# lppllppl920/EndoscopyDepthEstimation-Pytorch

Measured on AMD Instinct MI355X. Metric: train frame-pairs/sec at 256x320 bs=8, higher is better.
Workload: dtype f32

## Files before the change

### endoscopydepthestimation-pytorch_amd/csrc/conv_dma_kernels.h

```cpp
#pragma once

#include "conv_kernels.h"

namespace endo {

static __device__ __attribute__((aligned(16))) float g_pad_consts[8] = {__builtin_nanf(""), __builtin_nanf(""), __builtin_nanf(""), __builtin_nanf(""),
                                                                  0.0f, 0.0f, 0.0f, 0.0f};

typedef const __attribute__((address_space(1))) void* gptr_t;
typedef __attribute__((address_space(3))) void* lptr_t;

template <int KS, int KC, int Q, int WX, int R, int NBUF, int VEC, int IN = IN_PLAIN>
struct ConvDmaSmem {
    using G = ConvGeom<KS, KC, WX, R, VEC>;
    static constexpr int kW = KS * KS * KC * 16 * Q;
    static constexpr int kUG = (G::kTileX / 2) * (G::kTileY / 2);
    static constexpr int kUI = kUG / 4;
    static constexpr int kUStride = ((kUG + kUI - 8 + 31) / 32) * 32 + 8;
    static constexpr int kChan = (IN == IN_UNPOOL) ? kUStride : G::kCS;
    static constexpr int kBuf = KC * kChan + kW;
    static constexpr int kTail = 4 * 16 * Q + 8 * 16 * Q;
    static size_t bytes(int bn_cap) { return sizeof(float) * (NBUF * kBuf + 3 * bn_cap + kTail); }
};

template <int KS, int KC, int Q, int IN, int EPI, int WX, int R, int NBUF, int MINW, int VEC, int XF, int EXP = 0, int PH = -1, int BF = 0>
__global__ void __launch_bounds__(kConvThreads, MINW) conv_dma_kernel(const ConvParams p0) {
    static_assert(BF == 0 || (PH < 0 && (KS == 3 || KS == 1) && (IN == IN_BNRELU || IN == IN_PLAIN || (IN == IN_UNPOOL && KS == 1))),
                  "bf16 operands: the ordinary 3x3 convolution and the 1x1 convolutions of the transition-down layers");
    static_assert(PH < 0 || (KS == 3 && (Q % 2) == 0 && IN == IN_PLAIN && EPI == EPI_FWD), "phase mode is the transition-up forward");
    static_assert(IN != IN_UNPOOL || (KS == 1 && R % 2 == 0), "UNPOOL is the transition-down data gradient (1x1)");
    static_assert(NBUF == 1 || NBUF == 2, "one or two LDS buffers");
    static_assert(VEC == 1 || (VEC == 4 && IN != IN_UPSAMPLE && IN != IN_UNPOOL && IN != IN_SUBPIX), "16-byte DMA needs contiguous sources");
    static_assert(IN != IN_SUBPIX || (KS == 3 && EPI == EPI_FWD && PH < 0), "sub-pixel input mode is the transition-up data gradient");
    using G = ConvGeom<KS, KC, WX, R, VEC>;
    using S = ConvDmaSmem<KS, KC, Q, WX, R, NBUF, VEC, IN>;
    constexpr int KK = KS * KS;
    constexpr int NB = 16 * Q;
    constexpr int kWElems = S::kW;
    constexpr int kWPre = (kWElems + kConvThreads - 1) / kConvThreads;
    constexpr bool kDgrad = (EPI == EPI_DGRAD_BN || EPI == EPI_DGRAD_SUMPOOL);
    constexpr int kPhW = 2 * 12 * 16 + 16;
    static_assert(PH < 0 || KC * kPhW <= kWElems, "the phase weights fit the ordinary weight buffer");
    constexpr int kSubW = 4 * 16 * Q + 16;

    extern __shared__ __attribute__((aligned(16))) float smem[];
    float* s_aux = smem + NBUF * S::kBuf;
    int grp, n;
    group_of(p0, blockIdx.z, grp, n);
    const ConvParams p = group_view(p0, grp);
    const int groups = p0.group_n > 0 ? gridDim.z / p0.group_n : 1;
    const bool first_of_group = blockIdx.x == 0 && blockIdx.y == 0 && n == 0;
    (void)groups; (void)first_of_group;
    const int cap = p.bn_cap;

    const int tid = threadIdx.x;
    const int lane = tid & 63;
    const int wave = __builtin_amdgcn_readfirstlane(tid >> 6);
    const int tile = (gridDim.x & 7) == 0 ? xcd_remap(blockIdx.x, gridDim.x) : blockIdx.x;
    const int x0 = (tile % p.tiles_x) * G::kTileX;
    const int y0 = (tile / p.tiles_x) * G::kTileY;
    const int ph = PH == 2 ? static_cast<int>(blockIdx.y) : PH;
    const int co_base = (p.ksplit > 0 || PH == 2) ? 0 : blockIdx.y * NB;

    if constexpr (IN == IN_BNRELU) {
        for (int c = tid; c < p.cin; c += kConvThreads) {
            float scale, mean, beta;
            bn_input_constants(p, p0, grp, groups, first_of_group, c, scale, mean, beta);
            s_aux[c] = scale;
            s_aux[cap + c] = mean;
            s_aux[2 * cap + c] = beta;
        }
        for (int c = p.cin + tid; c < ((p.cin + KC - 1) / KC) * KC; c += kConvThreads) {
            s_aux[c] = 0.f; s_aux[cap + c] = 0.f; s_aux[2 * cap + c] = 0.f;
        }
    }
    if constexpr (EPI == EPI_DGRAD_BN) {
        float* cst = s_aux + 3 * cap;
        if (tid < NB) {
            const int c = co_base + tid;
            float mean = 0.f, rstd = 0.f, scale = 0.f, beta = 0.f;
            if (c < p.cout) {
                mean = p.bn_saved[2 * c];
                rstd = p.bn_saved[2 * c + 1];
                scale = p.bn_gamma[c] * rstd;
                beta = p.bn_beta[c];
            }
            cst[4 * tid] = scale; cst[4 * tid + 1] = beta; cst[4 * tid + 2] = mean; cst[4 * tid + 3] = rstd;
        }
    }

    f32x4 acc[R][Q];
#pragma unroll
    for (int r = 0; r < R; ++r)
#pragma unroll
        for (int q = 0; q < Q; ++q) acc[r][q] = f32x4{0.f, 0.f, 0.f, 0.f};

    const int wx = (wave % WX) * 16;
    const int wy = (wave / WX) * R;
    const int li = lane & 15;
    const int lk = lane >> 4;

    int goff[G::kPos];
    unsigned pos_ok = 0;
#pragma unroll
    for (int k = 0; k < G::kPos; ++k) {
        const int e = tid + k * kConvThreads;
        goff[k] = 0;
        if (e < G::kUnits) {
            const int ry = e / (G::kCols / VEC);
            const int rx = (e - ry * (G::kCols / VEC)) * VEC;
            const int gy = y0 - G::kHalo + ry;
            const int gx = x0 - G::kLeft + rx;
            if (gy >= 0 && gy < p.h && gx >= 0 && gx < p.w) {
                pos_ok |= (1u << k);
                if constexpr (IN == IN_UPSAMPLE) goff[k] = (gy >> 1) * p.in_w + (gx >> 1);
                else if constexpr (IN == IN_SUBPIX) goff[k] = 2 * gy * p.in_w + 2 * gx;
                else goff[k] = gy * p.in_w + gx;
            }
        }
    }
    constexpr int kUSlots = (IN == IN_UNPOOL) ? (KC * S::kUStride + kConvThreads - 1) / kConvThreads : 1;
    int uoff[kUSlots];
    if constexpr (IN == IN_UNPOOL) {
        constexpr int PC = G::kTileX / 2;
        const int ph = p.h >> 1, pw = p.w >> 1;
#pragma unroll
        for (int k = 0; k < kUSlots; ++k) {
            const int e = tid + k * kConvThreads;
            const int u = e % S::kUStride;
            int off = -1;
            if (e < KC * S::kUStride) {
                if (u < S::kUG) {
                    const int gy = (y0 >> 1) + u / PC, gx = (x0 >> 1) + u % PC;
                    if (gy < ph && gx < pw) off = gy * p.in_w + gx;
                } else if (u < S::kUG + S::kUI) {
                    const int q = u - S::kUG;
                    const int gy = (y0 >> 1) + q / (PC / 4), gx = (x0 >> 1) + 4 * (q % (PC / 4));
                    if (gy < ph && gx < pw) off = gy * p.in_w + gx;
                }
            }
            uoff[k] = off;
        }
    }
    const float* in_n = p.in + n * p.in_ns;
    const float* pad_in = g_pad_consts + (IN == IN_BNRELU ? 0 : 4);
    const float* pad_zero = g_pad_consts + 4;
    const int nchunks_all = (p.cin + KC - 1) / KC;
    int chunk_begin = 0, nchunks = nchunks_all;
    ConvParams po = p;
    if (p.ksplit > 0) {
        const int per = (nchunks_all + p.ksplit - 1) / p.ksplit;
        chunk_begin = blockIdx.y * per;
        nchunks = min(nchunks_all, chunk_begin + per);
        po.out = p.out + blockIdx.y * p.split_stride;
    }

    auto issue_dma = [&](int chunk, int buf) {
        const int c_base = chunk * KC;
        float* s_in = smem + buf * S::kBuf;
        float* s_w = s_in + KC * S::kChan;
        if constexpr (IN == IN_UNPOOL) {
            const uint8_t* idx_n = p.in_idx + n * p.idx_ns;
#pragma unroll
            for (int k = 0; k < kUSlots; ++k) {
                const int e0 = k * kConvThreads + wave * 64;
                if (e0 < KC * S::kUStride) {
                    const int e = e0 + lane;
                    const int ch = c_base + e / S::kUStride;
                    const bool is_code = (e % S::kUStride) >= S::kUG;
                    const void* src = pad_zero;
                    if (uoff[k] >= 0 && ch < p.cin) {
                        const int64_t o = static_cast<int64_t>(ch) * p.in_cs + uoff[k];
                        src = is_code ? static_cast<const void*>(idx_n + o) : static_cast<const void*>(in_n + o);
                    }
                    if (e < KC * S::kUStride) __builtin_amdgcn_global_load_lds((gptr_t)src, (lptr_t)(s_in + e0), 4, 0, 0);
                }
            }
        }
        int sub_ph = 0;
        if constexpr (IN == IN_SUBPIX) sub_ph = c_base / p.sub_c;
#pragma unroll
        for (int c = 0; c < (IN == IN_UNPOOL ? 0 : KC); ++c) {
            const int ch = c_base + c;
            const float* plane = in_n + static_cast<int64_t>(ch) * p.in_cs;
            if constexpr (IN == IN_SUBPIX)
                plane = in_n + static_cast<int64_t>(ch - sub_ph * p.sub_c) * p.in_cs + (sub_ph >> 1) * p.in_w + (sub_ph & 1);
#pragma unroll
            for (int k = 0; k < G::kPos; ++k) {
                const int e0 = k * kConvThreads + wave * 64;
                if (e0 < G::kUnits) {
                    const bool ok = (ch < p.cin) && (pos_ok & (1u << k));
                    const float* src = ok ? plane + goff[k] : pad_in;
                    if (e0 + lane < G::kUnits) {
                        if constexpr (VEC == 4)
                            __builtin_amdgcn_global_load_lds((gptr_t)src, (lptr_t)(s_in + c * G::kCS + 4 * e0), 16, 0, 0);
                        else
                            __builtin_amdgcn_global_load_lds((gptr_t)src, (lptr_t)(s_in + c * G::kCS + e0), 4, 0, 0);
                    }
                }
            }
        }
        if constexpr (IN == IN_SUBPIX) {
            constexpr int kUnitsW = KC * kSubW / 4;
            const float* wsrc = p.wgt + static_cast<int64_t>(c_base) * kSubW;
#pragma unroll
            for (int k = 0; k < (kUnitsW + kConvThreads - 1) / kConvThreads; ++k) {
                const int u0 = k * kConvThreads + wave * 64;
                if (u0 < kUnitsW && u0 + lane < kUnitsW)
                    __builtin_amdgcn_global_load_lds((gptr_t)(wsrc + 4 * (u0 + lane)), (lptr_t)(s_w + 4 * u0), 16, 0, 0);
            }
        }
        if constexpr (PH >= 0) {
            constexpr int kUnitsW = KC * kPhW / 4;
            const float* wsrc = p.wgt + static_cast<int64_t>(c_base) * kPhW + (PH == 2 ? static_cast<int64_t>(ph) * p.cin * 400 : 0);
#pragma unroll
            for (int k = 0; k < (kUnitsW + kConvThreads - 1) / kConvThreads; ++k) {
                const int u0 = k * kConvThreads + wave * 64;
                if (u0 < kUnitsW && u0 + lane < kUnitsW)
                    __builtin_amdgcn_global_load_lds((gptr_t)(wsrc + 4 * (u0 + lane)), (lptr_t)(s_w + 4 * u0), 16, 0, 0);
            }
        }
        constexpr bool kChunked = KS == 3 && KC == 16 && Q == 1 && EPI == EPI_FWD && PH < 0 && IN != IN_SUBPIX && BF == 0;
        bool gather = !(PH >= 0 || IN == IN_SUBPIX);
        if constexpr (kChunked) {
            if (p.wgt_chunks) {
                gather = false;
                constexpr int kUnitsW = kWElems / 4;
                const float* wsrc = p.wgt_chunks + static_cast<int64_t>(chunk) * kWElems;
#pragma unroll
                for (int k = 0; k < (kUnitsW + kConvThreads - 1) / kConvThreads; ++k) {
                    const int u0 = k * kConvThreads + wave * 64;
                    if (u0 < kUnitsW && u0 + lane < kUnitsW)
                        __builtin_amdgcn_global_load_lds((gptr_t)(wsrc + 4 * (u0 + lane)), (lptr_t)(s_w + 4 * u0), 16, 0, 0);
                }
            }
        }
        if (gather)
#pragma unroll
        for (int k = 0; k < ((PH >= 0 || IN == IN_SUBPIX) ? 0 : kWPre); ++k) {
            const int e0 = k * kConvThreads + wave * 64;
            if (e0 < kWElems) {
                const int e = e0 + lane;
                const int j = e % NB;
                const int rest = e / NB;
                const int c = rest % KC;
                const int tap = rest / KC;
                const int ci = c_base + c;
                const int co = co_base + j;
                const float* src = pad_zero;
                if (e < kWElems && ci < p.cin && co < (PH >= 0 ? p.w_cout : p.cout)) {
                    if constexpr (kDgrad) src = p.wgt + (static_cast<int64_t>(ci) * p.w_cin + co) * KK + (KK - 1 - tap);
                    else src = p.wgt + (static_cast<int64_t>(co) * p.w_cin + ci) * KK + tap;
                }
                if (e < kWElems) __builtin_amdgcn_global_load_lds((gptr_t)src, (lptr_t)(s_w + e0), 4, 0, 0);
            }
        }
    };

    constexpr int PR = (EPI == EPI_DGRAD_BN) ? R : 1, PQ = (EPI == EPI_DGRAD_BN) ? Q : 1;
    f32x4 xpre[PR][PQ], dpre[PR][PQ];
    bool use_pre = false;
    if constexpr (EPI == EPI_DGRAD_BN) {
        use_pre = ((p.out_w & 3) == 0) && ((p.w & 3) == 0);
        if (use_pre) {
            const int px = x0 + wx + 4 * lk;
#pragma unroll
            for (int q = 0; q < Q; ++q) {
                const int co = co_base + q * 16 + li;
#pragma unroll
                for (int r = 0; r < R; ++r) {
                    const int y = y0 + wy + r;
                    xpre[r][q] = f32x4{0.f, 0.f, 0.f, 0.f};
                    dpre[r][q] = f32x4{0.f, 0.f, 0.f, 0.f};
                    if (co < p.cout && y < p.h && px + 3 < p.w) {
                        xpre[r][q] = *reinterpret_cast<const f32x4*>(p.x + n * p.x_ns + static_cast<int64_t>(co) * p.x_cs + y * p.out_w + px);
                        if (co >= p.acc_from)
                            dpre[r][q] = *reinterpret_cast<const f32x4*>(p.out + n * p.out_ns + static_cast<int64_t>(co) * p.out_cs + y * p.out_w + px);
                    }
                }
            }
        }
    }

    constexpr bool kInPlace = (IN == IN_BNRELU) && (XF == 1);
    auto transform_own = [&](int chunk, int buf) {
        if constexpr (kInPlace) {
            float* s_in = smem + buf * S::kBuf;
#pragma unroll
            for (int c = 0; c < KC; ++c) {
                const int ch = chunk * KC + c;
                const float sc = s_aux[ch], mn = s_aux[cap + ch], bt = s_aux[2 * cap + ch];
#pragma unroll
                for (int k = 0; k < G::kPos; ++k) {
                    const int e = tid + k * kConvThreads;
                    if (e < G::kUnits) {
                        if constexpr (VEC == 4) {
                            f32x4* q = reinterpret_cast<f32x4*>(s_in + c * G::kCS + 4 * e);
                            f32x4 v = *q;
#pragma unroll
                            for (int i = 0; i < 4; ++i) v[i] = __builtin_fmaxf(fmaf(v[i] - mn, sc, bt), 0.f);
                            *q = v;
                        } else {
                            float* q = s_in + c * G::kCS + e;
                            *q = __builtin_fmaxf(fmaf(*q - mn, sc, bt), 0.f);
                        }
                    }
                }
            }
        }
    };

    auto compute = [&](int chunk, int buf) {
        const float* s_in = smem + buf * S::kBuf;
        const float* s_w = s_in + KC * S::kChan;
        int sub_alpha = 0, sub_beta = 0;
        if constexpr (IN == IN_SUBPIX) {
            const int sub_ph = (chunk * KC) / p.sub_c;
            sub_alpha = sub_ph >> 1; sub_beta = sub_ph & 1;
        }
        (void)sub_alpha; (void)sub_beta;
        if constexpr (IN == IN_UNPOOL) {
            constexpr int PC = G::kTileX / 2;
            const int pcol = (wx + li) >> 1;
            const unsigned sh = 8u * (pcol & 3);
            const unsigned want = li & 1;
            if constexpr (BF != 0) {
                constexpr int NQ = KC / 4;
#pragma unroll
                for (int qg = 0; qg < (NQ + 3) / 4; ++qg) {
                    float a[4][R], b[4][Q];
#pragma unroll
                    for (int i = 0; i < 4; ++i) {
                        const int quad = qg * 4 + i;
                        if (quad < NQ) {
                            const float* g_base = s_in + (quad * 4 + lk) * S::kUStride + (wy >> 1) * PC + pcol;
                            const unsigned* i_base = reinterpret_cast<const unsigned*>(s_in + (quad * 4 + lk) * S::kUStride + S::kUG);
                            const float* b_base = s_w + (quad * 4 + lk) * NB + li;
#pragma unroll
                            for (int rr = 0; rr < R / 2; ++rr) {
                                const float g = g_base[rr * PC];
                                const unsigned code = (i_base[(((wy >> 1) + rr) * PC + pcol) >> 2] >> sh) & 0xffu;
                                a[i][2 * rr] = code == want ? g : 0.f;
                                a[i][2 * rr + 1] = code == want + 2u ? g : 0.f;
                            }
#pragma unroll
                            for (int q = 0; q < Q; ++q) b[i][q] = b_base[q * 16];
                        } else {
#pragma unroll
                            for (int r = 0; r < R; ++r) a[i][r] = 0.f;
#pragma unroll
                            for (int q = 0; q < Q; ++q) b[i][q] = 0.f;
                        }
                    }
                    bf16x4_bits ap[R];
#pragma unroll
                    for (int r = 0; r < R; ++r) ap[r] = pack_bf16x4(a[0][r], a[1][r], a[2][r], a[3][r]);
#pragma unroll
                    for (int q = 0; q < Q; ++q) {
                        const bf16x4_bits bp = pack_bf16x4(b[0][q], b[1][q], b[2][q], b[3][q]);
#pragma unroll
                        for (int r = 0; r < R; ++r) acc[r][q] = __builtin_amdgcn_mfma_f32_16x16x16bf16_1k(ap[r], bp, acc[r][q], 0, 0, 0);
                    }
                }
                return;
            }
#pragma unroll
            for (int quad = 0; quad < KC / 4; ++quad) {
                const float* g_base = s_in + (quad * 4 + lk) * S::kUStride + (wy >> 1) * PC + pcol;
                const unsigned* i_base = reinterpret_cast<const unsigned*>(s_in + (quad * 4 + lk) * S::kUStride + S::kUG);
                const float* b_base = s_w + (quad * 4 + lk) * NB + li;
                float a[R];
#pragma unroll
                for (int rr = 0; rr < R / 2; ++rr) {
                    const float g = g_base[rr * PC];
                    const unsigned code = (i_base[(((wy >> 1) + rr) * PC + pcol) >> 2] >> sh) & 0xffu;
                    a[2 * rr] = code == want ? g : 0.f;
                    a[2 * rr + 1] = code == want + 2u ? g : 0.f;
                }
#pragma unroll
                for (int q = 0; q < Q; ++q) {
                    const float b = b_base[q * 16];
#pragma unroll
                    for (int r = 0; r < R; ++r) acc[r][q] = __builtin_amdgcn_mfma_f32_16x16x4f32(a[r], b, acc[r][q], 0, 0, 0);
                }
            }
            return;
        }
        if constexpr (BF != 0 && KS == 1) {
            constexpr int NQ = KC / 4;
#pragma unroll
            for (int qg = 0; qg < (NQ + 3) / 4; ++qg) {
                float a[4][R], b[4][Q];
#pragma unroll
                for (int i = 0; i < 4; ++i) {
                    const int quad = qg * 4 + i;
                    if (quad < NQ) {
                        const float* a_base = s_in + (quad * 4 + lk) * G::kCS + wy * G::kCols + wx + li + G::kColOff;
                        const float* b_base = s_w + (quad * 4 + lk) * NB + li;
                        float sc = 1.f, mn = 0.f, bt = 0.f;
                        if constexpr (IN == IN_BNRELU && !kInPlace) {
                            const int ch = chunk * KC + quad * 4 + lk;
                            sc = s_aux[ch]; mn = s_aux[cap + ch]; bt = s_aux[2 * cap + ch];
                        }
#pragma unroll
                        for (int r = 0; r < R; ++r) {
                            const float v = a_base[r * G::kCols];
                            a[i][r] = (IN == IN_BNRELU && !kInPlace) ? __builtin_fmaxf(fmaf(v - mn, sc, bt), 0.f) : v;
                        }
#pragma unroll
                        for (int q = 0; q < Q; ++q) b[i][q] = b_base[q * 16];
                    } else {
#pragma unroll
                        for (int r = 0; r < R; ++r) a[i][r] = 0.f;
#pragma unroll
                        for (int q = 0; q < Q; ++q) b[i][q] = 0.f;
                    }
                }
                bf16x4_bits ap[R];
#pragma unroll
                for (int r = 0; r < R; ++r) ap[r] = pack_bf16x4(a[0][r], a[1][r], a[2][r], a[3][r]);
#pragma unroll
                for (int q = 0; q < Q; ++q) {
                    const bf16x4_bits bp = pack_bf16x4(b[0][q], b[1][q], b[2][q], b[3][q]);
#pragma unroll
                    for (int r = 0; r < R; ++r) acc[r][q] = __builtin_amdgcn_mfma_f32_16x16x16bf16_1k(ap[r], bp, acc[r][q], 0, 0, 0);
                }
            }
            return;
        }
#pragma unroll
        for (int quad = 0; quad < KC / 4; ++quad) {
            const float* a_base = s_in + (quad * 4 + lk) * G::kCS + wy * G::kCols + wx + li + G::kColOff;
            const float* b_base = s_w + (quad * 4 + lk) * NB + li;
            float sc = 1.f, mn = 0.f, bt = 0.f;
            if constexpr (IN == IN_BNRELU && !kInPlace) {
                const int ch = chunk * KC + quad * 4 + lk;
                sc = s_aux[ch]; mn = s_aux[cap + ch]; bt = s_aux[2 * cap + ch];
            }
#pragma unroll
            for (int dx = 0; dx < KS; ++dx) {
                float a[R + KS - 1];
                if constexpr (BF != 0) {
#pragma unroll
                    for (int r = 0; r < R + 2; ++r) {
                        const float v = a_base[r * G::kCols + dx];
                        a[r] = (IN == IN_BNRELU && !kInPlace) ? __builtin_fmaxf(fmaf(v - mn, sc, bt), 0.f) : v;
                    }
                    bf16x4_bits ap[R];
#pragma unroll
                    for (int r = 0; r < R; ++r) ap[r] = pack_bf16x4(a[r], a[r + 1], a[r + 2], 0.f);
#pragma unroll
                    for (int q = 0; q < Q; ++q) {
                        const bf16x4_bits bp = pack_bf16x4(b_base[(0 * KS + dx) * KC * NB + q * 16], b_base[(1 * KS + dx) * KC * NB + q * 16],
                                                           b_base[(2 * KS + dx) * KC * NB + q * 16], 0.f);
#pragma unroll
                        for (int r = 0; r < R; ++r) acc[r][q] = __builtin_amdgcn_mfma_f32_16x16x16bf16_1k(ap[r], bp, acc[r][q], 0, 0, 0);
                    }
                    continue;
                }
                if constexpr (IN == IN_BNRELU && !kInPlace && !(EXP & 2)) {
                    typedef float f32x2 __attribute__((ext_vector_type(2)));
                    constexpr int NR = R + KS - 1;
                    const f32x2 mn2 = {mn, mn}, sc2 = {sc, sc}, bt2 = {bt, bt};
#pragma unroll
                    for (int r = 0; r + 1 < NR; r += 2) {
                        f32x2 v = {a_base[r * G::kCols + dx], a_base[(r + 1) * G::kCols + dx]};
                        v = __builtin_elementwise_fma(v - mn2, sc2, bt2);
                        a[r] = __builtin_fmaxf(v[0], 0.f);
                        a[r + 1] = __builtin_fmaxf(v[1], 0.f);
                    }
                    if constexpr (NR & 1) a[NR - 1] = __builtin_fmaxf(fmaf(a_base[(NR - 1) * G::kCols + dx] - mn, sc, bt), 0.f);
                } else {
#pragma unroll
                    for (int r = 0; r < R + KS - 1; ++r) a[r] = a_base[r * G::kCols + dx];
                }
                if constexpr (IN == IN_SUBPIX) {
                    if (dx == (sub_beta == 0 ? 0 : 2)) continue;
                }
#pragma unroll
                for (int dy = 0; dy < KS; ++dy) {
                    if (PH >= 0 && dy == (ph == 0 ? 2 : 0)) continue;
                    if constexpr (IN == IN_SUBPIX) {
                        if (dy == (sub_alpha == 0 ? 0 : 2)) continue;
                    }
#pragma unroll
                    for (int q = 0; q < Q; ++q) {
                        if (PH >= 0 && ((q < Q / 2 && dx == 2) || (q >= Q / 2 && dx == 0))) continue;
                        float b;
                        if constexpr (IN == IN_SUBPIX) {
                            const int tyi = dy - (sub_alpha == 0 ? 1 : 0), txi = dx - (sub_beta == 0 ? 1 : 0);
                            b = s_w[(quad * 4 + lk) * kSubW + (tyi * 2 + txi) * NB + q * 16 + li];
                        } else if constexpr (PH >= 0) {
                            const int slot = dx == 0 ? q : (dx == 1 ? Q / 2 + q : Q / 2 + Q + (q - Q / 2));
                            b = s_w[(quad * 4 + lk) * kPhW + ((dy - ph) * 2 * Q + slot) * 16 + li];
                        } else {
                            b = b_base[(dy * KS + dx) * KC * NB + q * 16];
                        }
#pragma unroll
                        for (int r = 0; r < R; ++r)
                            acc[r][q] = __builtin_amdgcn_mfma_f32_16x16x4f32(a[r + dy], b, acc[r][q], 0, 0, 0);
                    }
                }
            }
        }
    };

    issue_dma(chunk_begin, 0);
    if constexpr (kInPlace) {
        __syncthreads();
        asm volatile("s_waitcnt vmcnt(0)" ::: "memory");
        transform_own(chunk_begin, 0);
        __syncthreads();
        for (int chunk = chunk_begin; chunk < nchunks; ++chunk) {
            const int b = (chunk - chunk_begin) & 1;
            if (chunk + 1 < nchunks) issue_dma(chunk + 1, b ^ 1);
            compute(chunk, b);
            if (chunk + 1 < nchunks) {
                asm volatile("s_waitcnt vmcnt(0)" ::: "memory");
                transform_own(chunk + 1, b ^ 1);
            }
            __syncthreads();
        }
    } else {
        for (int chunk = chunk_begin; chunk < nchunks; ++chunk) {
            const int b = (chunk - chunk_begin) % NBUF;
            if (!(EXP & 4) || chunk == chunk_begin) asm volatile("s_waitcnt vmcnt(0)" ::: "memory");
            __syncthreads();
            if (NBUF == 2 && chunk + 1 < nchunks && !(EXP & 1)) issue_dma(chunk + 1, b ^ 1);
            compute(chunk, b);
            if (NBUF == 1 && chunk + 1 < nchunks) {
                __syncthreads();
                issue_dma(chunk + 1, 0);
            }
        }
    }

    if constexpr (EPI == EPI_DGRAD_BN) {
        if (use_pre) {
            const float* cst = s_aux + 3 * cap;
            float* s_red = s_aux + 3 * cap + 4 * NB;
            const int px = x0 + wx + 4 * lk;
#pragma unroll
            for (int q = 0; q < Q; ++q) {
                const int jloc = q * 16 + li;
                const int co = co_base + jloc;
                const float scale = cst[4 * jloc], beta = cst[4 * jloc + 1], mean = cst[4 * jloc + 2], rstd = cst[4 * jloc + 3];
                float s1 = 0.f, s2 = 0.f;
#pragma unroll
                for (int r = 0; r < R; ++r) {
                    const int y = y0 + wy + r;
                    if (co < p.cout && y < p.h && px + 3 < p.w) {
                        f32x4 o = dpre[r][q];
#pragma unroll
                        for (int e = 0; e < 4; ++e) {
                            const float xc = xpre[r][q][e] - mean;
                            const float z = fmaf(xc, scale, beta);
                            const float dz = z > 0.f ? acc[r][q][e] : 0.f;
                            s1 += dz;
                            s2 += dz * (xc * rstd);
                            o[e] += scale * dz;
                        }
                        *reinterpret_cast<f32x4*>(p.out + n * p.out_ns + static_cast<int64_t>(co) * p.out_cs + y * p.out_w + px) = o;
                    }
                }
                s1 += __shfl_xor(s1, 16, 64); s1 += __shfl_xor(s1, 32, 64);
                s2 += __shfl_xor(s2, 16, 64); s2 += __shfl_xor(s2, 32, 64);
                if (lk == 0) {
                    s_red[((tid >> 6) * NB + jloc) * 2] = s1;
                    s_red[((tid >> 6) * NB + jloc) * 2 + 1] = s2;
                }
            }
            __syncthreads();
            if (tid < 2 * NB) {
                const int j = tid >> 1, which = tid & 1;
                if (co_base + j < p.cout) {
                    double t = 0.0;
                    for (int wv = 0; wv < 4; ++wv) t += static_cast<double>(s_red[(wv * NB + j) * 2 + which]);
                    atomicAdd(p.bn_scratch + bn_slot_offset(p.bn_slot_stride) + 2 * (co_base + j) + which, t);
                }
            }
            return;
        }
    }
    if constexpr (PH >= 0) {
        constexpr int QH = Q / 2;
        float* s_red = s_aux + 3 * cap + 4 * NB;
        const int px = x0 + wx + 4 * lk;
#pragma unroll
        for (int q = 0; q < QH; ++q) {
            const int co = q * 16 + li;
            const bool co_ok = co < p.cout;
            const float bias = (co_ok && p.bias) ? p.bias[co] : 0.f;
            float s1 = 0.f, s2 = 0.f;
#pragma unroll
            for (int r = 0; r < R; ++r) {
                const int y = y0 + wy + r;
                if (co_ok && y < p.h && px + 3 < p.w) {
                    f32x4 lo, hi;
                    lo[0] = acc[r][q][0] + bias; lo[1] = acc[r][q + QH][0] + bias; lo[2] = acc[r][q][1] + bias; lo[3] = acc[r][q + QH][1] + bias;
                    hi[0] = acc[r][q][2] + bias; hi[1] = acc[r][q + QH][2] + bias; hi[2] = acc[r][q][3] + bias; hi[3] = acc[r][q + QH][3] + bias;
                    float* dst = p.out + n * p.out_ns + static_cast<int64_t>(co) * p.out_cs + static_cast<int64_t>(2 * y + ph) * p.out_w + 2 * px;
                    *reinterpret_cast<f32x4*>(dst) = lo;
                    *reinterpret_cast<f32x4*>(dst + 4) = hi;
#pragma unroll
                    for (int e = 0; e < 4; ++e) { s1 += lo[e] + hi[e]; s2 += lo[e] * lo[e] + hi[e] * hi[e]; }
                }
            }
            s1 += __shfl_xor(s1, 16, 64); s1 += __shfl_xor(s1, 32, 64);
            s2 += __shfl_xor(s2, 16, 64); s2 += __shfl_xor(s2, 32, 64);
            if (lk == 0) {
                s_red[((tid >> 6) * NB + q * 16 + li) * 2] = s1;
                s_red[((tid >> 6) * NB + q * 16 + li) * 2 + 1] = s2;
            }
        }
        __syncthreads();
        if (p.out_sums && tid < 2 * 16 * QH) {
            const int j = tid >> 1, which = tid & 1;
            if (j < p.cout) {
                double t = 0.0;
                for (int wv = 0; wv < 4; ++wv) t += static_cast<double>(s_red[(wv * NB + j) * 2 + which]);
                atomicAdd(p.out_sums + 2 * j + which, t);
            }
        }
        return;
    }
    conv_epilogue<Q, EPI, R>(po, acc, s_aux + 3 * cap, s_aux + 3 * cap + 4 * NB, x0, y0, wx, wy, co_base, n);
}

template <int KS, int KC, int Q, int IN, int EPI, int WX, int R, int NBUF, int MINW, int VEC, int XF = 0, int EXP = 0, int PH = -1, int BF = 0>
inline int launch_conv_dma_vec(ConvParams p, hipStream_t stream) {
    static_assert(XF == 0 || NBUF == 2 || IN != IN_BNRELU, "the in-place transform pipeline is written for two buffers");
    using G = ConvGeom<KS, KC, WX, R, VEC>;
    using S = ConvDmaSmem<KS, KC, Q, WX, R, NBUF, VEC, IN>;
    p.tiles_x = (p.w + G::kTileX - 1) / G::kTileX;
    p.bn_cap = (IN == IN_BNRELU) ? ((p.cin + KC - 1) / KC * KC + 15) / 16 * 16 : 0;
    const int tiles_y = (p.h + G::kTileY - 1) / G::kTileY;
    dim3 grid(p.tiles_x * tiles_y, p.ksplit > 0 ? p.ksplit : (PH >= 0 ? (PH == 2 ? 2 : 1) : (p.cout + 16 * Q - 1) / (16 * Q)), p.n);
    return launch_dyn(conv_dma_kernel<KS, KC, Q, IN, EPI, WX, R, NBUF, MINW, VEC, XF, EXP, PH, BF>, grid, kConvThreads, S::bytes(p.bn_cap), stream, p);
}

template <int KS, int KC, int Q, int IN, int EPI, int WX, int R, int NBUF, int MINW = 1, int BF = 0>
inline int launch_conv_dma(const ConvParams& p, hipStream_t stream) {
    if constexpr (IN != IN_UPSAMPLE && IN != IN_UNPOOL) {
        const bool aligned = (p.w % 4 == 0) && (p.in_w % 4 == 0) && (p.in_cs % 4 == 0) && (p.in_ns % 4 == 0) &&
                             (reinterpret_cast<uintptr_t>(p.in) % 16 == 0);
        if (aligned) return launch_conv_dma_vec<KS, KC, Q, IN, EPI, WX, R, NBUF, MINW, 4, 0, 0, -1, BF>(p, stream);
    }
    return launch_conv_dma_vec<KS, KC, Q, IN, EPI, WX, R, NBUF, MINW, 1, 0, 0, -1, BF>(p, stream);
}

template <int KS, int KC, int Q, int IN, int EPI, int BIG_R = 8, int NBUF = 2, int BIG_MINW = 1, int BF = 0>
inline int launch_conv_dma_auto(const ConvParams& p, hipStream_t stream) {
    const long tiles_big = static_cast<long>((p.w + 31) / 32) * ((p.h + 15) / 16) * p.n;
    if (tiles_big >= 512) return launch_conv_dma<KS, KC, Q, IN, EPI, 2, BIG_R, NBUF, BIG_MINW, BF>(p, stream);
    const long tiles_mid = static_cast<long>((p.w + 15) / 16) * ((p.h + 15) / 16) * p.n;
    if (tiles_mid >= 384) return launch_conv_dma<KS, KC, Q, IN, EPI, 1, 4, NBUF, 1, BF>(p, stream);
    constexpr int KCS = (NBUF == 2 && KS == 3 && KC <= 8) ? 16 : KC;
    return launch_conv_dma<KS, KCS, Q, IN, EPI, 1, 2, NBUF, 1, BF>(p, stream);
}

}
```

Baseline: 513.8.

## Pack multi-channel DMA loads for small split-K conv tiles; limit BN constant setup

For ksplit convolutions whose tile has at most 64 vector units per channel, input loads are packed across channels, so each wave issues full 64-lane global_load_lds transfers instead of partially filled per-channel ones. BN-ReLU input constants are now computed only for the channel slice a split block actually uses, not all input channels. Both changes aim to cut wasted DMA issue slots and redundant prologue work in small deep-layer convolutions. The packed path depends on the LDS channel stride equalling the plane size, and adds register pressure from the per-position offset arrays.

Result: no change. 514.5 (median of 6 runs) (+0.1%).

```diff
diff --git a/endoscopydepthestimation-pytorch_amd/csrc/conv_dma_kernels.h b/endoscopydepthestimation-pytorch_amd/csrc/conv_dma_kernels.h
--- a/endoscopydepthestimation-pytorch_amd/csrc/conv_dma_kernels.h
+++ b/endoscopydepthestimation-pytorch_amd/csrc/conv_dma_kernels.h
@@ -63,7 +63,13 @@
     const int co_base = (p.ksplit > 0 || PH == 2) ? 0 : blockIdx.y * NB;
 
     if constexpr (IN == IN_BNRELU) {
-        for (int c = tid; c < p.cin; c += kConvThreads) {
+        int c_lo = 0, c_hi = p.cin;
+        if (p.ksplit > 0 && !first_of_group) {
+            const int per = ((p.cin + KC - 1) / KC + p.ksplit - 1) / p.ksplit * KC;
+            c_lo = min(p.cin, static_cast<int>(blockIdx.y) * per);
+            c_hi = min(p.cin, c_lo + per);
+        }
+        for (int c = c_lo + tid; c < c_hi; c += kConvThreads) {
             float scale, mean, beta;
             bn_input_constants(p, p0, grp, groups, first_of_group, c, scale, mean, beta);
             s_aux[c] = scale;
@@ -119,6 +125,23 @@
             }
         }
     }
+    constexpr bool kPacked = VEC == 4 && KS == 3 && PH < 0 && XF == 0 && (IN == IN_PLAIN || IN == IN_BNRELU) && G::kUnits <= 64 && G::kCS == G::kPlane;
+    constexpr int kPackUnits = KC * G::kUnits;
+    constexpr int kPackPos = kPacked ? (kPackUnits + kConvThreads - 1) / kConvThreads : 1;
+    int pk_off[kPackPos], pk_ch[kPackPos];
+    if constexpr (kPacked) {
+#pragma unroll
+        for (int k = 0; k < kPackPos; ++k) {
+            const int e = tid + k * kConvThreads;
+            const int c = e / G::kUnits, u = e - c * G::kUnits;
+            const int ry = u / (G::kCols / VEC);
+            const int rx = (u - ry * (G::kCols / VEC)) * VEC;
+            const int gy = y0 - G::kHalo + ry;
+            const int gx = x0 - G::kLeft + rx;
+            pk_ch[k] = c;
+            pk_off[k] = (e < kPackUnits && gy >= 0 && gy < p.h && gx >= 0 && gx < p.w) ? c * p.in_cs + gy * p.in_w + gx : -1;
+        }
+    }
     constexpr int kUSlots = (IN == IN_UNPOOL) ? (KC * S::kUStride + kConvThreads - 1) / kConvThreads : 1;
     int uoff[kUSlots];
     if constexpr (IN == IN_UNPOOL) {
@@ -179,6 +202,20 @@
         }
         int sub_ph = 0;
         if constexpr (IN == IN_SUBPIX) sub_ph = c_base / p.sub_c;
+        const bool packed = kPacked && p.ksplit > 0;
+        if (packed) {
+            const float* first = in_n + static_cast<int64_t>(c_base) * p.in_cs;
+#pragma unroll
+            for (int k = 0; k < kPackPos; ++k) {
+                const int e0 = k * kConvThreads + wave * 64;
+                if (e0 < kPackUnits) {
+                    const bool ok = pk_off[k] >= 0 && c_base + pk_ch[k] < p.cin;
+                    const float* src = ok ? first + pk_off[k] : pad_in;
+                    if (e0 + lane < kPackUnits) __builtin_amdgcn_global_load_lds((gptr_t)src, (lptr_t)(s_in + 4 * e0), 16, 0, 0);
+                }
+            }
+        }
+        if (!packed)
 #pragma unroll
         for (int c = 0; c < (IN == IN_UNPOOL ? 0 : KC); ++c) {
             const int ch = c_base + c;
```
